# TaceoLabs/co-snarks

Hardware: NVIDIA H100
Metric: co-Groth16 proofs/sec (BN254, 2^20 constraints); MSM Mscalar/s (higher is better)
Workload: dtype u32x8 (256-bit Montgomery, integer)

## Files before the change

### co_snarks_b200/csrc/cs_groth16.cu

```cuda
#include <functional>
#include "cs_lib.cuh"
#include "cs_net.h"

using namespace cs;

struct cs_groth16_pk {
  int curve = 0;
  size_t nc = 0, ni = 0, nw = 0, n = 0;
  unsigned log_n = 0;
  DevBuf a_rowptr, a_col, a_coeff, b_rowptr, b_col, b_coeff;
  cs_bases *a_query = nullptr, *b_g1 = nullptr, *b_g2 = nullptr, *l_query = nullptr, *h_query = nullptr;
  std::vector<uint64_t> alpha_g1, beta_g1, beta_g2, delta_g1, delta_g2;
  std::vector<uint64_t> a_head, b1_head, b2_head;
  cs_domain* dom = nullptr;
  DevBuf coset_tab;
  DevBuf d_pub, d_wit, d_a, d_b, d_c, d_m1, d_m2;
  DevBuf c_rowptr, c_col, c_coeff;
  bool have_c = false;
  int wit_src[4] = {0, 1, 2, 3};
  cs_domain* dom_ark = nullptr;
  DevBuf coset_tab_ark, ginv_pows, vinv_over_n;
  DevBuf d_pt;
};

// ... 755 lines not shown

extern "C" {

int cs_groth16_rep3_prove(cs_ctx* ctx, cs_groth16_pk* pk, cs_net* net0, cs_net* net1, cs_rep3_state* state,
                          const uint64_t* h_pub, const uint64_t* h_wit, const uint64_t* d_wit, uint64_t* out_a,
                          uint64_t* out_b, uint64_t* out_c, uint64_t* out_rs) {
  return rep3_prove_dispatch(ctx, pk, net0, net1, nullptr, 0, state ? state->id : 0, state, h_pub, h_wit, d_wit, out_a, out_b,
                             out_c, out_rs);
}

int cs_groth16_rep3_prove_main(cs_ctx* ctx, cs_groth16_pk* pk, cs_net* net0, cs_net* net1, cs_net* pair,
                               cs_rep3_state* state, const uint64_t* h_pub, const uint64_t* h_wit, const uint64_t* d_wit,
                               uint64_t* out_a, uint64_t* out_b, uint64_t* out_c, uint64_t* out_rs) {
  return rep3_prove_dispatch(ctx, pk, net0, net1, pair, 1, state ? state->id : 0, state, h_pub, h_wit, d_wit, out_a, out_b,
                             out_c, out_rs);
}

int cs_groth16_rep3_prove_helper(cs_ctx* ctx, cs_groth16_pk* pk, int party, cs_net* pair, cs_rep3_state* state,
                                 const uint64_t* h_pub, const uint64_t* h_wit, const uint64_t* d_wit) {
  if (state && state->id != party) return fail(CS_ERR_ARG, "cs_groth16_rep3_prove_helper: state belongs to party %d", state->id);
  return rep3_prove_dispatch(ctx, pk, nullptr, nullptr, pair, 2, party, state, h_pub, h_wit, d_wit, nullptr, nullptr, nullptr,
                             nullptr);
}

int cs_groth16_pk_create(cs_ctx* ctx, const cs_groth16_key_desc* d, cs_groth16_pk** out) {
  return cs::groth16_pk_create(ctx, d, 0, out);
}

}

int cs::groth16_pk_create(cs_ctx* ctx, const cs_groth16_key_desc* d, unsigned k, cs_groth16_pk** out) {
  if (!ctx || !d || !out) return fail(CS_ERR_ARG, "cs_groth16_pk_create: NULL argument");
  if (d->curve != CS_BN254
#if defined(CS_ENABLE_BLS12_381)
      && d->curve != CS_BLS12_381
#endif
  )
    return fail(CS_ERR_ARG, "cs_groth16_pk_create: unsupported curve %d", (int)d->curve);
  const size_t nc = d->num_constraints, ni = d->num_instance_variables, nw = d->num_witness_variables;
  if (ni == 0) return fail(CS_ERR_ARG, "cs_groth16_pk_create: num_instance_variables must be >= 1");
  if (d->a_query_len != ni + nw || d->b_g1_query_len != ni + nw || d->b_g2_query_len != ni + nw)
    return fail(CS_ERR_ARG, "cs_groth16_pk_create: a/b query length must be %zu", ni + nw);
  if (d->l_query_len != nw) return fail(CS_ERR_ARG, "cs_groth16_pk_create: l_query length must be %zu", nw);
  if (d->window_bits && (d->window_bits < 2 || d->window_bits > (int)MSM_MAX_WINDOW))
    return fail(CS_ERR_ARG, "cs_bases_upload: window_bits %d out of range [2,%u] (0 = automatic)", d->window_bits, MSM_MAX_WINDOW);
  CS_CUDA(cudaSetDevice(ctx->device));
  std::unique_ptr<cs_groth16_pk, void (*)(cs_groth16_pk*)> pk(new cs_groth16_pk(), cs_groth16_pk_free);
  pk->curve = d->curve;
  pk->nc = nc; pk->ni = ni; pk->nw = nw;
  size_t n = 1;
  unsigned lg = 0;
  while (n < nc + ni) { n <<= 1; lg++; }
  pk->n = n;
  pk->log_n = lg;
  if (d->h_query_len < n) return fail(CS_ERR_ARG, "cs_groth16_pk_create: h_query has %zu points, domain needs %zu", d->h_query_len, n);
  const unsigned max_adicity = d->curve == CS_BN254 ? 28 : 32;
  if (lg > max_adicity) return fail(CS_ERR_ARG, "Polynomial Degree too large");
  const size_t fq = fq_limbs64(d->curve), g1b = 2 * fq * 8, g2b = 4 * fq * 8;
  CS_TRY(upload(ctx, pk->a_rowptr, d->a_row_ptr, (nc + 1) * 4));
  CS_TRY(upload(ctx, pk->a_col, d->a_col, d->a_nnz * 4));
  CS_TRY(upload(ctx, pk->a_coeff, d->a_coeff, d->a_nnz * 32));
  CS_TRY(upload(ctx, pk->b_rowptr, d->b_row_ptr, (nc + 1) * 4));
  CS_TRY(upload(ctx, pk->b_col, d->b_col, d->b_nnz * 4));
  CS_TRY(upload(ctx, pk->b_coeff, d->b_coeff, d->b_nnz * 32));
  if (d->c_row_ptr) {
    CS_TRY(upload(ctx, pk->c_rowptr, d->c_row_ptr, (nc + 1) * 4));
    CS_TRY(upload(ctx, pk->c_col, d->c_col, d->c_nnz * 4));
    CS_TRY(upload(ctx, pk->c_coeff, d->c_coeff, d->c_nnz * 32));
    pk->have_c = true;
  }
  CS_CUDA(cudaStreamSynchronize(ctx->stream));
  pk->alpha_g1.assign(d->alpha_g1, d->alpha_g1 + 2 * fq);
  pk->beta_g1.assign(d->beta_g1, d->beta_g1 + 2 * fq);
  pk->beta_g2.assign(d->beta_g2, d->beta_g2 + 4 * fq);
  pk->delta_g1.assign(d->delta_g1, d->delta_g1 + 2 * fq);
  pk->delta_g2.assign(d->delta_g2, d->delta_g2 + 4 * fq);
  pk->a_head.assign(d->a_query, d->a_query + ni * 2 * fq);
  pk->b1_head.assign(d->b_g1_query, d->b_g1_query + ni * 2 * fq);
  pk->b2_head.assign(d->b_g2_query, d->b_g2_query + ni * 4 * fq);
  (void)g1b; (void)g2b;
  const int wb = d->window_bits;
  int wwb = wb, hwb = wb;
  CS_DISPATCH_CURVE(d->curve, {
    if (!wwb) wwb = (int)msm_auto_window(nw, Cfg::FR_BITS);
    if (!hwb) hwb = (int)msm_auto_window(n, Cfg::FR_BITS);
    const unsigned cmax = wwb > hwb ? wwb : hwb;
    const unsigned W = msm_shape(Cfg::FR_BITS, wwb < hwb ? wwb : hwb).W;
    if (!k)
      CS_TRY(pick_table_rows(ctx, cmax, W, [&](unsigned kk) { return key_bytes<Cfg>(ni, nw, n, wwb, hwb, kk); },
                             "cs_groth16_pk_create", &k));
  });
  CS_TRY(bases_upload(ctx, d->curve, CS_G1, d->a_query, d->a_query_len, wwb, k, &pk->a_query));
  CS_TRY(bases_upload(ctx, d->curve, CS_G1, d->b_g1_query, d->b_g1_query_len, wwb, k, &pk->b_g1));
  CS_TRY(bases_upload(ctx, d->curve, CS_G2, d->b_g2_query, d->b_g2_query_len, wwb, k, &pk->b_g2));
  if (nw) CS_TRY(bases_upload(ctx, d->curve, CS_G1, d->l_query, d->l_query_len, wwb, k, &pk->l_query));
  CS_TRY(bases_upload(ctx, d->curve, CS_G1, d->h_query, n, hwb, k, &pk->h_query));
  CS_TRY(plan_witness_views(ctx, pk.get()));
  switch (d->curve) {
    case CS_BN254: CS_TRY(build_coset_table<Bn254Cfg>(ctx, pk.get())); break;
#if defined(CS_ENABLE_BLS12_381)
    case CS_BLS12_381: CS_TRY(build_coset_table<Bls381Cfg>(ctx, pk.get())); break;
#endif
    default: break;
  }
  *out = pk.release();
  return 0;
}

extern "C" {

void cs_groth16_pk_free(cs_groth16_pk* pk) {
  if (!pk) return;
  DevBuf* bufs[] = {&pk->a_rowptr, &pk->a_col, &pk->a_coeff, &pk->b_rowptr, &pk->b_col, &pk->b_coeff, &pk->coset_tab,
                    &pk->d_pub, &pk->d_wit, &pk->d_a, &pk->d_b, &pk->d_c, &pk->d_m1, &pk->d_m2,
                    &pk->c_rowptr, &pk->c_col, &pk->c_coeff, &pk->coset_tab_ark, &pk->ginv_pows, &pk->vinv_over_n,
                    &pk->d_pt};
  for (DevBuf* b : bufs) b->release();
  cs_bases_free(pk->a_query);
  cs_bases_free(pk->b_g1);
  cs_bases_free(pk->b_g2);
  cs_bases_free(pk->l_query);
  cs_bases_free(pk->h_query);
  cs_domain_free(pk->dom);
  cs_domain_free(pk->dom_ark);
  delete pk;
}

size_t cs_groth16_domain_size(const cs_groth16_pk* pk) { return pk ? pk->n : 0; }

int cs_groth16_pk_table_info(const cs_groth16_pk* pk, unsigned* table_rows, size_t* table_bytes) {
  if (!pk) return fail(CS_ERR_ARG, "cs_groth16_pk_table_info: pk is NULL");
  const cs_bases* q[5] = {pk->a_query, pk->b_g1, pk->b_g2, pk->l_query, pk->h_query};
  size_t bytes = 0;
  for (const cs_bases* b : q)
    if (b) bytes += b->table.cap + b->infmask.cap;
  if (table_rows) *table_rows = pk->a_query->sh.T;
  if (table_bytes) *table_bytes = bytes;
  return 0;
}
int cs_groth16_pk_curve(const cs_groth16_pk* pk) { return pk ? pk->curve : CS_ERR_ARG; }

int cs_groth16_witness_map(cs_ctx* ctx, cs_groth16_pk* pk, cs_share_kind kind, int party, const uint64_t* h_pub,
                           const uint64_t* h_wit, const uint64_t* h_m1, const uint64_t* h_m2, uint64_t* h_out) {
  if (!ctx || !pk || !h_pub || (pk->nw && !h_wit)) return fail(CS_ERR_ARG, "cs_groth16_witness_map: NULL argument");
  if (kind != CS_PLAIN && kind != CS_REP3) return fail(CS_ERR_ARG, "cs_groth16_witness_map: bad share kind");
  if (kind == CS_REP3 && (party < 0 || party > 2)) return fail(CS_ERR_ARG, "cs_groth16_witness_map: party must be 0..2");
  CS_CUDA(cudaSetDevice(ctx->device));
  CS_TRY(upload_inputs(ctx, pk, kind, h_pub, h_wit, h_m1, h_m2));
  switch (pk->curve) {
    case CS_BN254:
      CS_TRY((witness_map_device<Bn254Cfg>(ctx, pk, kind, party, pk->d_wit.as<uint32_t>(), h_m1 != nullptr,
                                           h_m2 != nullptr, ctx->stream)));
      break;
#if defined(CS_ENABLE_BLS12_381)
    case CS_BLS12_381:
      CS_TRY((witness_map_device<Bls381Cfg>(ctx, pk, kind, party, pk->d_wit.as<uint32_t>(), h_m1 != nullptr,
                                            h_m2 != nullptr, ctx->stream)));
      break;
#endif
    default: return fail(CS_ERR_ARG, "unsupported curve");
  }
  if (h_out) CS_CUDA(cudaMemcpyAsync(h_out, pk->d_c.p, pk->n * 32, cudaMemcpyDeviceToHost, ctx->stream));
  CS_CUDA(cudaStreamSynchronize(ctx->stream));
  return 0;
}

int cs_groth16_witness_map_libsnark(cs_ctx* ctx, cs_groth16_pk* pk, cs_share_kind kind, int party, const uint64_t* h_pub,
                                    const uint64_t* h_wit, const uint64_t* h_mask, uint64_t* h_out) {
// ... 187 lines not shown
```

### co_snarks_b200/csrc/cs_msm.cuh

```cuda
#pragma once
#include <stdlib.h>
#include "cs_common.cuh"
#include "cs_curve.cuh"

namespace cs {

constexpr unsigned MSM_SLICE_MAX = 64;
constexpr unsigned MSM_ORDER_BLOCK = 256;
constexpr unsigned MSM_RED_SEG = 4;
constexpr unsigned MSM_SIGN = 0x80000000u;

template <class FrP, class Fn>
CS_D void msm_recode(const uint32_t* __restrict__ scalars, uint32_t sstride, uint32_t i, int mont, uint32_t c,
                     uint32_t W, uint32_t k, Fn&& f) {
  Fp<FrP> s;
  const uint4* src = reinterpret_cast<const uint4*>(scalars) + (size_t)i * sstride * (FrP::N / 4);
  CS_UNROLL
  for (int q = 0; q < FrP::N / 4; q++) {
    uint4 v = src[q];
    s.l[4 * q] = v.x; s.l[4 * q + 1] = v.y; s.l[4 * q + 2] = v.z; s.l[4 * q + 3] = v.w;
  }
  if (mont) s = s.from_mont();
  const uint32_t half = 1u << (c - 1);
  const uint32_t mask = (1u << c) - 1;
  uint32_t carry = 0, row = 0, gb = 0;
  for (uint32_t w = 0; w < W; w++) {
    uint32_t pos = w * c;
    uint32_t li = pos >> 5, sh = pos & 31;
    uint32_t lo = li < FrP::N ? s.l[li] : 0;
    uint32_t hi = li + 1 < FrP::N ? s.l[li + 1] : 0;
    uint32_t d = (__funnelshift_r(lo, hi, sh) & mask) + carry;
    uint32_t out;
    if (d > half) {
      out = ((1u << c) - d) | MSM_SIGN;
      carry = 1;
    } else {
      out = d;
      carry = 0;
    }
    f(row, out & ~MSM_SIGN ? out + gb : 0);
    gb += half;
    if (gb == k * half) {
      gb = 0;
      row++;
    }
  }
}

CS_D bool msm_base_inf(const uint32_t* __restrict__ infmask, uint32_t k) {
  return infmask && ((infmask[k >> 5] >> (k & 31)) & 1);
}

constexpr unsigned MSM_BIN_T = 1024;
constexpr unsigned MSM_BIN_TILE = 4096;
constexpr unsigned MSM_BIN_SPAN = 1u << 15;
constexpr unsigned MSM_SCATTER_SPAN = 1u << 13;

template <class FrP>
CS_GLOBAL void __launch_bounds__(MSM_BIN_T) k_msm_bin_count(const uint32_t* __restrict__ scalars, uint32_t sstride,
                                                            uint32_t n, int mont, uint32_t c, uint32_t W, uint32_t kw,
                                                            const uint32_t* __restrict__ infmask, uint32_t offset,
                                                            uint32_t tile, uint32_t nblk_p, uint32_t pstride, uint32_t B,
                                                            uint32_t* __restrict__ tab) {
  CS_DYN_SMEM(uint32_t, h);
  const uint32_t bt = blockIdx.x % nblk_p;
  scalars += (size_t)(blockIdx.x / nblk_p) * pstride * FrP::N;
  const uint32_t lo = blockIdx.y * MSM_BIN_SPAN + 1;
  const uint32_t span = B + 1 - lo < MSM_BIN_SPAN ? B + 1 - lo : MSM_BIN_SPAN;
  for (uint32_t k = threadIdx.x; k < span; k += blockDim.x) h[k] = 0;
  __syncthreads();
  const uint32_t i1 = (bt + 1) * tile < n ? (bt + 1) * tile : n;
  for (uint32_t i = bt * tile + threadIdx.x; i < i1; i += blockDim.x) {
    if (msm_base_inf(infmask, offset + i)) continue;
    msm_recode<FrP>(scalars, sstride, i, mont, c, W, kw, [&](uint32_t, uint32_t d) {
      const uint32_t k = (d & ~MSM_SIGN) - lo;
      if (k < span) atomicAdd(&h[k], 1u);
    });
  }
  __syncthreads();
  uint32_t* row = tab + (size_t)blockIdx.x * B + (lo - 1);
  for (uint32_t k = threadIdx.x; k < span; k += blockDim.x) row[k] = h[k];
}

constexpr unsigned MSM_BIN_SCAN_U = 16;
static CS_GLOBAL void k_msm_bin_scan(uint32_t* __restrict__ tab, uint32_t nblk, uint32_t B, uint32_t NB,
                                     uint32_t* __restrict__ count) {
  const uint32_t b = blockIdx.x * blockDim.x + threadIdx.x;
  if (b == 0) count[0] = 0;
  if (b >= NB) return;
  uint32_t* col = tab + (size_t)(b / B) * nblk * B + b % B;
  uint32_t run = 0, r = 0;
  for (; r + MSM_BIN_SCAN_U <= nblk; r += MSM_BIN_SCAN_U) {
    uint32_t v[MSM_BIN_SCAN_U];
    CS_UNROLL
    for (uint32_t u = 0; u < MSM_BIN_SCAN_U; u++) v[u] = col[(size_t)(r + u) * B];
    CS_UNROLL
    for (uint32_t u = 0; u < MSM_BIN_SCAN_U; u++) {
      col[(size_t)(r + u) * B] = run;
      run += v[u];
    }
  }
  for (; r < nblk; r++) {
    const uint32_t v = col[(size_t)r * B];
    col[(size_t)r * B] = run;
    run += v;
  }
  count[b + 1] = run;
}

template <class FrP>
CS_GLOBAL void __launch_bounds__(MSM_BIN_T) k_msm_bin_scatter(const uint32_t* __restrict__ scalars, uint32_t sstride,
                                                              uint32_t n, int mont, uint32_t c, uint32_t W, uint32_t kw,
                                                              const uint32_t* __restrict__ infmask, uint32_t offset,
                                                              uint32_t tile, uint32_t nblk_p, uint32_t pstride,
                                                              uint32_t B, uint32_t nbases,
                                                              const uint32_t* __restrict__ tab,
                                                              const uint32_t* __restrict__ start,
                                                              uint32_t* __restrict__ sorted) {
  CS_DYN_SMEM(uint32_t, cur);
  const uint32_t p = blockIdx.x / nblk_p, bt = blockIdx.x % nblk_p;
  scalars += (size_t)p * pstride * FrP::N;
  const uint32_t lo = blockIdx.y * MSM_SCATTER_SPAN + 1;
  const uint32_t span = B + 1 - lo < MSM_SCATTER_SPAN ? B + 1 - lo : MSM_SCATTER_SPAN;
  const uint32_t* row = tab + (size_t)blockIdx.x * B + (lo - 1);
  for (uint32_t k = threadIdx.x; k < span; k += blockDim.x) cur[k] = start[p * B + lo + k] + row[k];
  __syncthreads();
  const uint32_t i1 = (bt + 1) * tile < n ? (bt + 1) * tile : n;
  for (uint32_t i = bt * tile + threadIdx.x; i < i1; i += blockDim.x) {
    if (msm_base_inf(infmask, offset + i)) continue;
    msm_recode<FrP>(scalars, sstride, i, mont, c, W, kw, [&](uint32_t row, uint32_t d) {
      const uint32_t k = (d & ~MSM_SIGN) - lo;
      if (k < span) sorted[atomicAdd(&cur[k], 1u)] = (row * nbases + offset + i) | (d & MSM_SIGN);
    });
  }
}

template <class F>
CS_GLOBAL void k_msm_infmask(const Affine<F>* __restrict__ table, uint32_t n, uint32_t* __restrict__ mask) {
  uint32_t wd = blockIdx.x * blockDim.x + threadIdx.x;
  if (wd * 32 >= n) return;
  uint32_t m = 0;
  for (uint32_t k = 0; k < 32 && wd * 32 + k < n; k++)
    if (table[wd * 32 + k].is_inf()) m |= 1u << k;
  mask[wd] = m;
}

constexpr unsigned MSM_SCAN_T = 1024;
constexpr unsigned MSM_SCAN_MAX_BLOCKS = 1024;
CS_D void msm_scan_terms(const uint32_t* __restrict__ count, uint32_t k, uint32_t nb1, uint32_t S, uint32_t* v) {
  uint32_t cnt = (k && k < nb1) ? count[k] : 0;
  uint32_t n0 = (cnt + S - 1) / S;
  uint32_t n1 = (n0 + S - 1) / S;
  v[0] = cnt; v[1] = n0; v[2] = n1; v[3] = (n1 + S - 1) / S;
}
static CS_GLOBAL void k_msm_scan1(const uint32_t* __restrict__ count, uint32_t nb1 , uint32_t S,
                                  uint32_t* __restrict__ start, uint32_t* __restrict__ sstart0,
                                  uint32_t* __restrict__ sstart1, uint32_t* __restrict__ sstart2, uint32_t* __restrict__ aux) {
  __shared__ uint32_t sm[4][32];
  const uint32_t t = threadIdx.x, lane = t & 31, wid = t >> 5, nwarp = blockDim.x >> 5;
  const uint32_t k = blockIdx.x * blockDim.x + t;
  uint32_t v[4], inc[4];
  msm_scan_terms(count, k, nb1, S, v);
  CS_UNROLL
  for (int q = 0; q < 4; q++) {
    uint32_t x = v[q];
    CS_UNROLL
    for (uint32_t d = 1; d < 32; d <<= 1) {
      uint32_t y = __shfl_up_sync(0xffffffffu, x, d);
      if (lane >= d) x += y;
    }
    inc[q] = x;
    if (lane == 31) sm[q][wid] = x;
  }
  __syncthreads();
  uint32_t w[4], x[4];
  CS_UNROLL
  for (int q = 0; q < 4; q++) {
    w[q] = (wid == 0 && lane < nwarp) ? sm[q][lane] : 0;
    x[q] = w[q];
    CS_UNROLL
    for (uint32_t d = 1; d < 32; d <<= 1) {
      uint32_t y = __shfl_up_sync(0xffffffffu, x[q], d);
      if (lane >= d) x[q] += y;
    }
  }
  __syncthreads();
  if (wid == 0 && lane < nwarp) {
    CS_UNROLL
    for (int q = 0; q < 4; q++) sm[q][lane] = x[q] - w[q];
    if (lane == nwarp - 1) {
      CS_UNROLL
      for (int q = 0; q < 4; q++) aux[blockIdx.x * 4 + q] = x[q];
    }
  }
  __syncthreads();
  if (k < nb1) {
    start[k] = sm[0][wid] + inc[0] - v[0];
    sstart0[k] = sm[1][wid] + inc[1] - v[1];
    sstart1[k] = sm[2][wid] + inc[2] - v[2];
    sstart2[k] = sm[3][wid] + inc[3] - v[3];
  }
}
static CS_GLOBAL void k_msm_scan2(const uint32_t* __restrict__ count, uint32_t nb1, uint32_t S,
                                  uint32_t* __restrict__ start, uint32_t* __restrict__ sstart0,
                                  uint32_t* __restrict__ sstart1, uint32_t* __restrict__ sstart2,
                                  const uint32_t* __restrict__ aux) {
  const uint32_t k = blockIdx.x * blockDim.x + threadIdx.x;
  if (k >= nb1) return;
  uint32_t off[4] = {0, 0, 0, 0};
  for (uint32_t b = 0; b < blockIdx.x; b++) {
    CS_UNROLL
    for (int q = 0; q < 4; q++) off[q] += aux[b * 4 + q];
  }
  uint32_t a = start[k] + off[0], b0 = sstart0[k] + off[1], b1 = sstart1[k] + off[2], b2 = sstart2[k] + off[3];
  start[k] = a; sstart0[k] = b0; sstart1[k] = b1; sstart2[k] = b2;
  if (k == nb1 - 1) {
    uint32_t v[4];
    msm_scan_terms(count, k, nb1, S, v);
    start[nb1] = a + v[0]; sstart0[nb1] = b0 + v[1]; sstart1[nb1] = b1 + v[2]; sstart2[nb1] = b2 + v[3];
  }
}

constexpr unsigned MSM_VIEW_T = 256;
constexpr unsigned MSM_VIEW_WORDS = MSM_VIEW_T / 32;

CS_D uint32_t popc32(uint32_t x) {
#if defined(CS_EMU)
  return (uint32_t)__builtin_popcount(x);
#else
  return __popc(x);
#endif
// ... 390 lines not shown

constexpr uint32_t POINT_INV_RUN = 32;

template <class F, class FrP>
CS_GLOBAL void __launch_bounds__(128) k_point_terms(const Affine<F>* __restrict__ base, const uint32_t* __restrict__ scalars,
                                                    uint32_t nterms, Xyzz<F>* __restrict__ prod) {
  const uint32_t t = blockIdx.x * blockDim.x + threadIdx.x;
  if (t >= nterms) return;
  Fp<FrP> s;
  CS_UNROLL
  for (int k = 0; k < FrP::N; k++) s.l[k] = scalars[(size_t)t * FrP::N + k];
  prod[t] = scalar_mul<F, FrP>(base[t], s.from_mont());
}

template <class F>
CS_GLOBAL void __launch_bounds__(128) k_point_sum(const Xyzz<F>* __restrict__ prod, uint32_t T, uint32_t nout,
                                                  const Xyzz<F>* __restrict__ add0, const Xyzz<F>* __restrict__ add1,
                                                  const Affine<F>* __restrict__ shared, Xyzz<F>* __restrict__ out) {
  const uint32_t o = blockIdx.x * blockDim.x + threadIdx.x;
  if (o >= nout) return;
  Xyzz<F> acc = shared ? Xyzz<F>::from_affine(*shared) : Xyzz<F>::inf();
  for (uint32_t j = 0; j < T + 2; j++) {
    const Xyzz<F>* q = j < T ? prod + (size_t)o * T + j : (j == T ? add0 : add1);
    if (q && j >= T) q += o;
    if (q) padd(acc, *q);
  }
  out[o] = acc;
}

template <class F>
CS_GLOBAL void __launch_bounds__(128) k_point_affine(const Xyzz<F>* __restrict__ in, uint32_t nout, uint32_t ostride,
                                                     Affine<F>* __restrict__ out) {
  const uint32_t lo = (blockIdx.x * blockDim.x + threadIdx.x) * POINT_INV_RUN;
  if (lo >= nout) return;
  const uint32_t hi = lo + POINT_INV_RUN < nout ? lo + POINT_INV_RUN : nout;
  F run = F::one();
  for (uint32_t o = lo; o < hi; o++) {
    if (!in[o].is_inf()) run = run * in[o].zzz;
    out[(size_t)o * ostride].x = run;
  }
  F inv = run.inverse();
  for (uint32_t o = hi; o-- > lo;) {
    Affine<F> a = Affine<F>::inf();
    if (!in[o].is_inf()) {
      const F zi = o > lo ? inv * out[(size_t)(o - 1) * ostride].x : inv;
      inv = inv * in[o].zzz;
      const F zzi = (zi * in[o].zz).sqr();
      a.x = in[o].x * zzi;
      a.y = in[o].y * zi;
    }
    out[(size_t)o * ostride] = a;
  }
}

struct MsmShape {
  uint32_t c, W, B;
  uint32_t k = 1, T = 0;
  uint32_t nb() const { return k * B; }
};

static inline MsmShape msm_shape(uint32_t scalar_bits, uint32_t c, uint32_t k = 1) {
  MsmShape s;
  s.c = c;
  s.W = (scalar_bits + 1 + c - 1) / c;
  s.B = 1u << (c - 1);
  s.k = k < s.W ? k : s.W;
  s.T = (s.W + s.k - 1) / s.k;
  return s;
}

static inline uint32_t msm_auto_window(size_t n, uint32_t scalar_bits) {
  int lg = 0;
  while ((1ull << (lg + 1)) <= n) lg++;
  int c = lg >= 15 ? 16 : lg - 4;
  if (c < 4) c = 4;
  while (c < 16) {
    const uint32_t W = (scalar_bits + 1 + c - 1) / c;
    const uint32_t top = scalar_bits + 1 - (W - 1) * c;
    if (2 * top >= (uint32_t)c) break;
    c++;
  }
  return (uint32_t)c;
}
static inline uint32_t msm_slice(const MsmShape& sh) {
  const char* e = getenv("CS_MSM_SLICE");
  if (e && atoi(e) == 64) return 64u;
  if (e && atoi(e) == 32) return 32u;
  return sh.c >= 18 ? 64u : 32u;
}

constexpr int MSM_NSTAGE = 5;
struct MsmWorkspace {
  DevBuf dig, sorted, meta, part0, part1, part2, bucket, red, scal, result, order;
  void* h_result = nullptr;
  size_t h_result_cap = 0;
  bool profile = false;
  cudaEvent_t ev[MSM_NSTAGE + 1] = {};
  cudaEvent_t sorted_ev = nullptr;
  bool sorted_ev_made = false, sorted_once = false;
  cudaEvent_t acc_in = nullptr, acc_out = nullptr;
  size_t bytes() const {
    return dig.cap + sorted.cap + meta.cap + part0.cap + part1.cap + part2.cap + bucket.cap + red.cap + scal.cap +
           result.cap + order.cap;
  }
  int mark(int i, cudaStream_t st) {
    if (!profile) return 0;
    if (!ev[i]) CS_CUDA(cudaEventCreateWithFlags(&ev[i], 0));
    CS_CUDA(cudaEventRecord(ev[i], st));
    return 0;
  }
  void release() {
    for (int i = 0; i <= MSM_NSTAGE; i++) {
      if (ev[i]) cudaEventDestroy(ev[i]);
      ev[i] = nullptr;
    }
    if (sorted_ev_made) cudaEventDestroy(sorted_ev);
    if (acc_in) cudaEventDestroy(acc_in);
    if (acc_out) cudaEventDestroy(acc_out);
    acc_in = acc_out = nullptr;
    sorted_ev = nullptr;
    sorted_ev_made = sorted_once = false;
    dig.release(); sorted.release(); meta.release(); part0.release(); part1.release(); part2.release();
    bucket.release(); red.release(); scal.release(); result.release(); order.release();
    if (h_result) cudaFreeHost(h_result);
    h_result = nullptr;
    h_result_cap = 0;
  }
};

template <class F>
int msm_accum0_f52(const Affine<F>* table, const uint32_t* sorted, const uint32_t* count, const uint32_t* start,
                   const uint32_t* sstart0, uint32_t nb1, uint32_t S, const uint32_t* order, const uint32_t* order_b,
                   Xyzz<F>* part0, uint32_t max_s0, cudaStream_t st);

struct MsmSizes {
  uint32_t nb1, S, ob, K;
  size_t nent, max_s0, max_s1, max_s2;
  MsmSizes(const MsmShape& sh, uint32_t n, uint32_t K_ = 1) {
    K = K_;
    nb1 = K * sh.nb() + 1;
    nent = (size_t)K * sh.W * n;
    S = msm_slice(sh);
    max_s0 = nent / S + nb1;
    max_s1 = max_s0 / S + nb1;
    max_s2 = max_s1 / S + nb1;
    ob = ceil_div(max_s0, MSM_ORDER_BLOCK);
  }
  size_t meta_words() const { return (size_t)nb1 + 4 * ((size_t)nb1 + 1) + 4 * MSM_SCAN_MAX_BLOCKS; }
  size_t order_words() const {
    return 4 * max_s0 + (size_t)ob * (MSM_SLICE_MAX + 1) + 2 * (MSM_SLICE_MAX + 1) + (size_t)(MSM_SLICE_MAX + 1) * MSM_OFF_CHUNKS;
  }
};
struct MsmSortBufs {
  uint32_t *count, *start, *sstart0, *sstart1, *sstart2, *aux;
  uint32_t *slice_len, *slice_bkt, *order, *order_b, *block_hist, *len_base, *chunk_sum;
  MsmSortBufs(const MsmWorkspace& w, const MsmSizes& z) {
    count = w.meta.as<uint32_t>();
    start = count + z.nb1;
    sstart0 = start + z.nb1 + 1;
    sstart1 = sstart0 + z.nb1 + 1;
    sstart2 = sstart1 + z.nb1 + 1;
    aux = sstart2 + z.nb1 + 1;
    slice_len = w.order.as<uint32_t>();
    slice_bkt = slice_len + z.max_s0;
    order = slice_bkt + z.max_s0;
    order_b = order + z.max_s0;
    block_hist = order_b + z.max_s0;
    len_base = block_hist + (size_t)z.ob * (MSM_SLICE_MAX + 1);
    chunk_sum = len_base + 2 * (MSM_SLICE_MAX + 1);
  }
};

static inline uint32_t msm_max_batch(const MsmShape& sh, uint32_t n) {
  size_t K = ((size_t)MSM_SCAN_MAX_BLOCKS * MSM_SCAN_T - 1) / sh.nb();
  if (n) K = K < ((1ull << 31) - 1) / ((size_t)sh.W * n) ? K : ((1ull << 31) - 1) / ((size_t)sh.W * n);
  K = K < 65535 / sh.k ? K : 65535 / sh.k;
  return (uint32_t)K;
}

static inline int msm_check_limits(const MsmShape& sh, uint32_t n, uint32_t nbases, uint32_t K = 1) {
  const size_t nent = (size_t)K * sh.W * n;
  if (nent >= (1ull << 31) || (size_t)sh.T * nbases >= (1ull << 31))
    return fail(-3, "msm: K*W*n = %zu entries or T*nbases = %zu table slots exceed 2^31", nent, (size_t)sh.T * nbases);
  if (K > 1 && K > msm_max_batch(sh, n))
    return fail(-3, "msm: a batch of %u MSMs exceeds the %u that one sort takes in this window shape (K*k*B + 1 <= 2^20 "
                    "buckets, K*k <= 65535 groups)", K, msm_max_batch(sh, n));
  return 0;
}

static inline int msm_scan(const MsmSortBufs& q, const MsmSizes& z, uint32_t NB, cudaStream_t st) {
  const uint32_t sb = ceil_div(z.nb1, MSM_SCAN_T);
  if (sb > MSM_SCAN_MAX_BLOCKS) return fail(-3, "msm: %u buckets exceed the scan's limit", NB);
  CS_LAUNCH_SYNC(k_msm_scan1, sb, MSM_SCAN_T, 0, st, q.count, z.nb1, z.S, q.start, q.sstart0, q.sstart1, q.sstart2, q.aux);
  CS_LAUNCH(k_msm_scan2, sb, MSM_SCAN_T, 0, st, q.count, z.nb1, z.S, q.start, q.sstart0, q.sstart1, q.sstart2, q.aux);
  return 0;
}

static inline int msm_slice_order(MsmWorkspace& ws, const MsmSortBufs& q, const MsmSizes& z, cudaStream_t st) {
  CS_LAUNCH_SYNC(k_msm_slice_hist, z.ob, MSM_ORDER_BLOCK, 0, st, q.count, q.sstart0, z.nb1, z.S, q.slice_len, q.slice_bkt,
                 q.block_hist);
  const uint32_t nt = (MSM_SLICE_MAX + 1) * MSM_OFF_CHUNKS;
  CS_LAUNCH(k_msm_slice_off1, ceil_div(nt, 128), 128, 0, st, q.block_hist, z.ob, q.chunk_sum);
  CS_LAUNCH(k_msm_slice_off2, 1, 128, 0, st, q.chunk_sum, q.len_base);
  CS_LAUNCH(k_msm_slice_off3, ceil_div(nt, 128), 128, 0, st, q.block_hist, z.ob, q.chunk_sum, q.len_base);
  CS_LAUNCH_SYNC(k_msm_slice_order, z.ob, MSM_ORDER_BLOCK, 0, st, q.slice_len, q.slice_bkt, (uint32_t)z.max_s0, q.sstart0,
                 z.nb1, q.block_hist, q.len_base, q.order, q.order_b);
  if (!ws.sorted_ev_made) {
    CS_CUDA(cudaEventCreateWithFlags(&ws.sorted_ev, cudaEventDisableTiming));
    ws.sorted_ev_made = true;
  }
  CS_CUDA(cudaEventRecord(ws.sorted_ev, st));
  ws.sorted_once = true;
  return 0;
}

template <class FrP>
int msm_smem_optin() {
#if !defined(CS_EMU)
  CS_CUDA(cudaFuncSetAttribute(k_msm_bin_count<FrP>, cudaFuncAttributeMaxDynamicSharedMemorySize, MSM_BIN_SPAN * 4));
  CS_CUDA(cudaFuncSetAttribute(k_msm_bin_scatter<FrP>, cudaFuncAttributeMaxDynamicSharedMemorySize, MSM_SCATTER_SPAN * 4));
#endif
  return 0;
}

static inline uint32_t msm_bin_tile(const MsmShape& sh, const MsmSizes& z, uint32_t n) {
  const size_t ent = z.nent / z.K;
  const size_t rows = ent / sh.nb() > 1 ? ent / sh.nb() : 1;
  const size_t nblk = ceil_div(n, MSM_BIN_TILE) < rows ? ceil_div(n, MSM_BIN_TILE) : rows;
  return n ? ceil_div(n, nblk) : 1;
}

static inline size_t msm_sort_dig_words(const MsmShape& sh, const MsmSizes& z, uint32_t n) {
  const size_t tab_words = (size_t)z.K * (n ? ceil_div(n, msm_bin_tile(sh, z, n)) : 0) * sh.nb();
  return tab_words > z.nent ? tab_words : z.nent;
}
static inline size_t msm_view_dig_words(const MsmSizes& z) {
  const size_t nblk = ceil_div(z.nent, MSM_VIEW_T);
  return nblk * MSM_VIEW_WORDS + 2 * nblk + 1;
}

template <class F>
struct MsmReduce {
  uint32_t L, nseg_g, nseg, ngroups, fs_threads, fs_blocks;
  size_t red_elems;
  explicit MsmReduce(const MsmShape& sh, uint32_t K = 1) {
    L = sh.B < MSM_RED_SEG ? sh.B : MSM_RED_SEG;
    nseg_g = sh.B / L;
    ngroups = K * sh.k;
    nseg = ngroups * nseg_g;
    fs_threads = sizeof(Xyzz<F>) > 128 ? 128 : 256;
    fs_blocks = nseg_g > 4 * fs_threads ? (nseg_g + fs_threads - 1) / fs_threads : 1;
    red_elems = (size_t)nseg + (size_t)ngroups * fs_blocks + (sh.k > 1 ? ngroups : 0);
  }
};

static inline size_t msm_sort_bytes(const MsmShape& sh, uint32_t n, uint32_t K = 1) {
  const MsmSizes z(sh, n, K);
  const size_t dig = msm_sort_dig_words(sh, z, n) > msm_view_dig_words(z) ? msm_sort_dig_words(sh, z, n) : msm_view_dig_words(z);
  return DevBuf::alloc_size(dig * 4) + DevBuf::alloc_size(z.nent * 4) + DevBuf::alloc_size(z.meta_words() * 4) +
         DevBuf::alloc_size(z.order_words() * 4);
}
template <class F>
size_t msm_accum_bytes(const MsmShape& sh, uint32_t n, uint32_t K = 1) {
  const MsmSizes z(sh, n, K);
  const size_t x = sizeof(Xyzz<F>);
  return DevBuf::alloc_size(z.max_s0 * x) + DevBuf::alloc_size(z.max_s1 * x) + DevBuf::alloc_size(z.max_s2 * x) +
         DevBuf::alloc_size((size_t)z.nb1 * x) + DevBuf::alloc_size(MsmReduce<F>(sh, K).red_elems * x) +
         DevBuf::alloc_size(K * x);
}

template <class FrP>
int msm_sort(MsmWorkspace& ws, const uint32_t* infmask, uint32_t nbases, MsmShape sh, uint32_t offset,
             const uint32_t* d_scalars, uint32_t sstride, uint32_t n, int mont, cudaStream_t st, uint32_t K = 1,
             uint32_t pstride = 0) {
  CS_TRY(msm_check_limits(sh, n, nbases, K));
  const MsmSizes z(sh, n, K);
  const uint32_t tile = msm_bin_tile(sh, z, n);
  const uint32_t nblk_p = n ? ceil_div(n, tile) : 0, nblk = K * nblk_p;
  const uint32_t NB = sh.nb();
  const dim3 grid(nblk, ceil_div(NB, MSM_BIN_SPAN)), grid_sc(nblk, ceil_div(NB, MSM_SCATTER_SPAN));
  const uint32_t smem = (NB < MSM_BIN_SPAN ? NB : MSM_BIN_SPAN) * 4;
  const uint32_t smem_sc = (NB < MSM_SCATTER_SPAN ? NB : MSM_SCATTER_SPAN) * 4;
  CS_TRY(ws.dig.reserve(msm_sort_dig_words(sh, z, n) * 4));
  CS_TRY(ws.sorted.reserve(z.nent * 4));
  CS_TRY(ws.meta.reserve(z.meta_words() * 4));
  CS_TRY(ws.order.reserve(z.order_words() * 4));
  const MsmSortBufs q(ws, z);
  uint32_t* tab = ws.dig.as<uint32_t>();
  CS_TRY(ws.mark(0, st));
  if (nblk)
    CS_LAUNCH_SYNC(k_msm_bin_count<FrP>, grid, MSM_BIN_T, smem, st, d_scalars, sstride, n, mont, sh.c, sh.W, sh.k,
                   infmask, offset, tile, nblk_p, pstride, NB, tab);
  CS_TRY(ws.mark(1, st));
  CS_LAUNCH(k_msm_bin_scan, ceil_div(K * NB, 256), 256, 0, st, tab, nblk_p, NB, K * NB, q.count);
  CS_TRY(msm_scan(q, z, K * NB, st));
  if (nblk)
    CS_LAUNCH_SYNC(k_msm_bin_scatter<FrP>, grid_sc, MSM_BIN_T, smem_sc, st, d_scalars, sstride, n, mont, sh.c, sh.W, sh.k,
                   infmask, offset, tile, nblk_p, pstride, NB, nbases, tab, q.start, ws.sorted.as<uint32_t>());
  return msm_slice_order(ws, q, z, st);
}

static inline int msm_view(MsmWorkspace& ws, const MsmWorkspace& src, const uint32_t* infmask, uint32_t nbases,
                           MsmShape sh, uint32_t offset, uint32_t n, cudaStream_t st, uint32_t K = 1) {
  const MsmSizes z(sh, n, K);
  const uint32_t nblk = ceil_div(z.nent, MSM_VIEW_T);
  CS_TRY(ws.dig.reserve(msm_view_dig_words(z) * 4));
  CS_TRY(ws.sorted.reserve(z.nent * 4));
  CS_TRY(ws.meta.reserve(z.meta_words() * 4));
  CS_TRY(ws.order.reserve(z.order_words() * 4));
  const MsmSortBufs q(ws, z), s(src, z);
  uint32_t* keep = ws.dig.as<uint32_t>();
  uint32_t* blk_cnt = keep + (size_t)nblk * MSM_VIEW_WORDS;
  uint32_t* blk_off = blk_cnt + nblk;
  const uint32_t* src_sorted = src.sorted.as<uint32_t>();
  CS_LAUNCH_SYNC(k_msm_view_flags, nblk, MSM_VIEW_T, 0, st, src_sorted, s.start, z.nb1, n, infmask, offset, keep, blk_cnt);
  CS_LAUNCH_SYNC(k_msm_view_scan, 1, MSM_SCAN_T, 0, st, blk_cnt, nblk, blk_off);
  CS_LAUNCH(k_msm_view_counts, ceil_div(z.nb1, 256), 256, 0, st, s.start, z.nb1, keep, blk_off, q.count);
  CS_LAUNCH(k_msm_view_scatter, nblk, MSM_VIEW_T, 0, st, src_sorted, n, nbases, offset, keep, blk_off,
            ws.sorted.as<uint32_t>());
  CS_TRY(msm_scan(q, z, K * sh.nb(), st));
  return msm_slice_order(ws, q, z, st);
}

template <class F, class FrP>
int msm_enqueue(MsmWorkspace& ws, const Affine<F>* table, const uint32_t* infmask, uint32_t nbases, MsmShape sh,
                uint32_t offset,
                const uint32_t* d_scalars, uint32_t sstride, uint32_t n, int mont, cudaStream_t st,
                MsmWorkspace* sort_from = nullptr, bool view = false, bool table_m260 = false, cudaStream_t st_acc = nullptr,
                uint32_t K = 1, uint32_t pstride = 0) {
  CS_TRY(msm_check_limits(sh, n, nbases, K));
  const MsmSizes z(sh, n, K);
  const uint32_t nb1 = z.nb1, S = z.S;
  const size_t max_s0 = z.max_s0, max_s1 = z.max_s1, max_s2 = z.max_s2;
  CS_TRY(ws.part0.reserve(max_s0 * sizeof(Xyzz<F>)));
  CS_TRY(ws.part1.reserve(max_s1 * sizeof(Xyzz<F>)));
  CS_TRY(ws.part2.reserve(max_s2 * sizeof(Xyzz<F>)));
  CS_TRY(ws.bucket.reserve((size_t)nb1 * sizeof(Xyzz<F>)));
  const MsmReduce<F> rd(sh, K);
  const uint32_t L = rd.L, nseg = rd.nseg, fs_threads = rd.fs_threads, fs_blocks = rd.fs_blocks, G = rd.ngroups;
  CS_TRY(ws.red.reserve(rd.red_elems * sizeof(Xyzz<F>)));
  CS_TRY(ws.result.reserve(K * sizeof(Xyzz<F>)));
  if (ws.h_result_cap < K * sizeof(Xyzz<F>)) {
    if (ws.h_result) cudaFreeHost(ws.h_result);
    ws.h_result = nullptr;
    ws.h_result_cap = 0;
    CS_CUDA(cudaMallocHost(&ws.h_result, K * sizeof(Xyzz<F>)));
    ws.h_result_cap = K * sizeof(Xyzz<F>);
  }
  if (sort_from) {
    if (!sort_from->sorted_once) return fail(-1, "msm: the workspace to share a sort with has not been enqueued");
    CS_TRY(ws.mark(0, st));
    CS_CUDA(cudaStreamWaitEvent(st, sort_from->sorted_ev, 0));
    CS_TRY(ws.mark(1, st));
    if (view) CS_TRY(msm_view(ws, *sort_from, infmask, nbases, sh, offset, n, st, K));
  } else {
    CS_TRY(msm_sort<FrP>(ws, infmask, nbases, sh, offset, d_scalars, sstride, n, mont, st, K, pstride));
  }
  MsmWorkspace& so = sort_from && !view ? *sort_from : ws;
  const MsmSortBufs q(so, z);
  const uint32_t *count = q.count, *start = q.start, *sstart0 = q.sstart0, *sstart1 = q.sstart1, *sstart2 = q.sstart2;
  const uint32_t *order = q.order, *order_b = q.order_b;
  CS_TRY(ws.mark(2, st));
  cudaStream_t st_main = st;
  if (st_acc) {
    if (!ws.acc_in) {
      CS_CUDA(cudaEventCreateWithFlags(&ws.acc_in, cudaEventDisableTiming));
      CS_CUDA(cudaEventCreateWithFlags(&ws.acc_out, cudaEventDisableTiming));
    }
    CS_CUDA(cudaEventRecord(ws.acc_in, st));
    CS_CUDA(cudaStreamWaitEvent(st_acc, ws.acc_in, 0));
    st = st_acc;
  }
  {
    static int minb_env = -1;
    if (minb_env < 0) { const char* e = getenv("CS_ACCUM0_MINB"); minb_env = e ? atoi(e) : 0; }
    const int minb = minb_env ? minb_env : (sizeof(Affine<F>) > 64 ? 2 : 4);
    if (table_m260) {
      CS_TRY((msm_accum0_f52<F>(table, so.sorted.as<uint32_t>(), count, start, sstart0, nb1, S, order, order_b,
                                ws.part0.as<Xyzz<F>>(), (uint32_t)max_s0, st)));
    } else {
#define CS_ACC0(M)                                                                                              \
// ... 47 lines not shown
```

Measured before the change: 51.66.

## Use 17-bit MSM windows for large keys with 16-bit packed bin counters

For key MSMs of at least 2^18 points where auto-selection picks c=16, the window becomes 17 bits when that reduces the window count. For BN254 this means 15 windows instead of 16. To fit the doubled bucket range in shared memory, the bin count kernel packs two 16-bit counters per word, with the tile capped so counts cannot overflow. The scatter span, scan block limit and reduction segment length are also widened to handle more buckets. The trade is fewer windows and bucket passes against larger bucket reductions, bigger precomputed tables and more shared-memory atomics contention.

```diff
diff --git a/co_snarks_b200/csrc/cs_groth16.cu b/co_snarks_b200/csrc/cs_groth16.cu
--- a/co_snarks_b200/csrc/cs_groth16.cu
+++ b/co_snarks_b200/csrc/cs_groth16.cu
@@ -861,8 +861,8 @@
   const int wb = d->window_bits;
   int wwb = wb, hwb = wb;
   CS_DISPATCH_CURVE(d->curve, {
-    if (!wwb) wwb = (int)msm_auto_window(nw, Cfg::FR_BITS);
-    if (!hwb) hwb = (int)msm_auto_window(n, Cfg::FR_BITS);
+    if (!wwb) wwb = (int)msm_key_window(nw, Cfg::FR_BITS);
+    if (!hwb) hwb = (int)msm_key_window(n, Cfg::FR_BITS);
     const unsigned cmax = wwb > hwb ? wwb : hwb;
     const unsigned W = msm_shape(Cfg::FR_BITS, wwb < hwb ? wwb : hwb).W;
     if (!k)
diff --git a/co_snarks_b200/csrc/cs_msm.cuh b/co_snarks_b200/csrc/cs_msm.cuh
--- a/co_snarks_b200/csrc/cs_msm.cuh
+++ b/co_snarks_b200/csrc/cs_msm.cuh
@@ -8,6 +8,7 @@
 constexpr unsigned MSM_SLICE_MAX = 64;
 constexpr unsigned MSM_ORDER_BLOCK = 256;
 constexpr unsigned MSM_RED_SEG = 4;
+constexpr unsigned MSM_RED_MAX_SEG = 1u << 13;
 constexpr unsigned MSM_SIGN = 0x80000000u;
 
 template <class FrP, class Fn>
@@ -54,32 +55,40 @@
 constexpr unsigned MSM_BIN_T = 1024;
 constexpr unsigned MSM_BIN_TILE = 4096;
 constexpr unsigned MSM_BIN_SPAN = 1u << 15;
+constexpr unsigned MSM_BIN_SPAN16 = 1u << 16;
 constexpr unsigned MSM_SCATTER_SPAN = 1u << 13;
+constexpr unsigned MSM_SCATTER_SPAN_MAX = 1u << 14;
+
+static inline uint32_t msm_scatter_span(uint32_t NB) { return NB > MSM_BIN_SPAN ? MSM_SCATTER_SPAN_MAX : MSM_SCATTER_SPAN; }
 
 template <class FrP>
 CS_GLOBAL void __launch_bounds__(MSM_BIN_T) k_msm_bin_count(const uint32_t* __restrict__ scalars, uint32_t sstride,
                                                             uint32_t n, int mont, uint32_t c, uint32_t W, uint32_t kw,
                                                             const uint32_t* __restrict__ infmask, uint32_t offset,
                                                             uint32_t tile, uint32_t nblk_p, uint32_t pstride, uint32_t B,
-                                                            uint32_t* __restrict__ tab) {
+                                                            uint32_t h16, uint32_t* __restrict__ tab) {
   CS_DYN_SMEM(uint32_t, h);
   const uint32_t bt = blockIdx.x % nblk_p;
   scalars += (size_t)(blockIdx.x / nblk_p) * pstride * FrP::N;
-  const uint32_t lo = blockIdx.y * MSM_BIN_SPAN + 1;
-  const uint32_t span = B + 1 - lo < MSM_BIN_SPAN ? B + 1 - lo : MSM_BIN_SPAN;
-  for (uint32_t k = threadIdx.x; k < span; k += blockDim.x) h[k] = 0;
+  const uint32_t hspan = h16 ? MSM_BIN_SPAN16 : MSM_BIN_SPAN;
+  const uint32_t lo = blockIdx.y * hspan + 1;
+  const uint32_t span = B + 1 - lo < hspan ? B + 1 - lo : hspan;
+  for (uint32_t k = threadIdx.x; k < (h16 ? (span + 1) >> 1 : span); k += blockDim.x) h[k] = 0;
   __syncthreads();
   const uint32_t i1 = (bt + 1) * tile < n ? (bt + 1) * tile : n;
   for (uint32_t i = bt * tile + threadIdx.x; i < i1; i += blockDim.x) {
     if (msm_base_inf(infmask, offset + i)) continue;
     msm_recode<FrP>(scalars, sstride, i, mont, c, W, kw, [&](uint32_t, uint32_t d) {
       const uint32_t k = (d & ~MSM_SIGN) - lo;
-      if (k < span) atomicAdd(&h[k], 1u);
+      if (k < span) {
+        if (h16) atomicAdd(&h[k >> 1], 1u << ((k & 1) << 4));
+        else atomicAdd(&h[k], 1u);
+      }
     });
   }
   __syncthreads();
   uint32_t* row = tab + (size_t)blockIdx.x * B + (lo - 1);
-  for (uint32_t k = threadIdx.x; k < span; k += blockDim.x) row[k] = h[k];
+  for (uint32_t k = threadIdx.x; k < span; k += blockDim.x) row[k] = h16 ? (h[k >> 1] >> ((k & 1) << 4)) & 0xffffu : h[k];
 }
 
 constexpr unsigned MSM_BIN_SCAN_U = 16;
@@ -113,15 +122,15 @@
                                                               uint32_t n, int mont, uint32_t c, uint32_t W, uint32_t kw,
                                                               const uint32_t* __restrict__ infmask, uint32_t offset,
                                                               uint32_t tile, uint32_t nblk_p, uint32_t pstride,
-                                                              uint32_t B, uint32_t nbases,
+                                                              uint32_t B, uint32_t nbases, uint32_t sspan,
                                                               const uint32_t* __restrict__ tab,
                                                               const uint32_t* __restrict__ start,
                                                               uint32_t* __restrict__ sorted) {
   CS_DYN_SMEM(uint32_t, cur);
   const uint32_t p = blockIdx.x / nblk_p, bt = blockIdx.x % nblk_p;
   scalars += (size_t)p * pstride * FrP::N;
-  const uint32_t lo = blockIdx.y * MSM_SCATTER_SPAN + 1;
-  const uint32_t span = B + 1 - lo < MSM_SCATTER_SPAN ? B + 1 - lo : MSM_SCATTER_SPAN;
+  const uint32_t lo = blockIdx.y * sspan + 1;
+  const uint32_t span = B + 1 - lo < sspan ? B + 1 - lo : sspan;
   const uint32_t* row = tab + (size_t)blockIdx.x * B + (lo - 1);
   for (uint32_t k = threadIdx.x; k < span; k += blockDim.x) cur[k] = start[p * B + lo + k] + row[k];
   __syncthreads();
@@ -146,7 +155,7 @@
 }
 
 constexpr unsigned MSM_SCAN_T = 1024;
-constexpr unsigned MSM_SCAN_MAX_BLOCKS = 1024;
+constexpr unsigned MSM_SCAN_MAX_BLOCKS = 2048;
 CS_D void msm_scan_terms(const uint32_t* __restrict__ count, uint32_t k, uint32_t nb1, uint32_t S, uint32_t* v) {
   uint32_t cnt = (k && k < nb1) ? count[k] : 0;
   uint32_t n0 = (cnt + S - 1) / S;
@@ -703,6 +712,12 @@
   }
   return (uint32_t)c;
 }
+
+static inline uint32_t msm_key_window(size_t n, uint32_t scalar_bits) {
+  const uint32_t c = msm_auto_window(n, scalar_bits);
+  if (n < (1u << 18) || c != 16) return c;
+  return (scalar_bits + 1 + 16) / 17 < (scalar_bits + 1 + 15) / 16 ? 17u : 16u;
+}
 static inline uint32_t msm_slice(const MsmShape& sh) {
   const char* e = getenv("CS_MSM_SLICE");
   if (e && atoi(e) == 64) return 64u;
@@ -804,7 +819,7 @@
   if (nent >= (1ull << 31) || (size_t)sh.T * nbases >= (1ull << 31))
     return fail(-3, "msm: K*W*n = %zu entries or T*nbases = %zu table slots exceed 2^31", nent, (size_t)sh.T * nbases);
   if (K > 1 && K > msm_max_batch(sh, n))
-    return fail(-3, "msm: a batch of %u MSMs exceeds the %u that one sort takes in this window shape (K*k*B + 1 <= 2^20 "
+    return fail(-3, "msm: a batch of %u MSMs exceeds the %u that one sort takes in this window shape (K*k*B + 1 <= 2^21 "
                     "buckets, K*k <= 65535 groups)", K, msm_max_batch(sh, n));
   return 0;
 }
@@ -839,16 +854,19 @@
 int msm_smem_optin() {
 #if !defined(CS_EMU)
   CS_CUDA(cudaFuncSetAttribute(k_msm_bin_count<FrP>, cudaFuncAttributeMaxDynamicSharedMemorySize, MSM_BIN_SPAN * 4));
-  CS_CUDA(cudaFuncSetAttribute(k_msm_bin_scatter<FrP>, cudaFuncAttributeMaxDynamicSharedMemorySize, MSM_SCATTER_SPAN * 4));
+  CS_CUDA(cudaFuncSetAttribute(k_msm_bin_scatter<FrP>, cudaFuncAttributeMaxDynamicSharedMemorySize, MSM_SCATTER_SPAN_MAX * 4));
 #endif
   return 0;
 }
+
+static inline bool msm_count16(const MsmShape& sh) { return sh.nb() > MSM_BIN_SPAN && sh.nb() <= MSM_BIN_SPAN16; }
 
 static inline uint32_t msm_bin_tile(const MsmShape& sh, const MsmSizes& z, uint32_t n) {
   const size_t ent = z.nent / z.K;
   const size_t rows = ent / sh.nb() > 1 ? ent / sh.nb() : 1;
   const size_t nblk = ceil_div(n, MSM_BIN_TILE) < rows ? ceil_div(n, MSM_BIN_TILE) : rows;
-  return n ? ceil_div(n, nblk) : 1;
+  const uint32_t tile = n ? ceil_div(n, nblk) : 1;
+  return msm_count16(sh) && tile > 65535 / sh.T ? 65535 / sh.T : tile;
 }
 
 static inline size_t msm_sort_dig_words(const MsmShape& sh, const MsmSizes& z, uint32_t n) {
@@ -865,7 +883,7 @@
   uint32_t L, nseg_g, nseg, ngroups, fs_threads, fs_blocks;
   size_t red_elems;
   explicit MsmReduce(const MsmShape& sh, uint32_t K = 1) {
-    L = sh.B < MSM_RED_SEG ? sh.B : MSM_RED_SEG;
+    L = sh.B < MSM_RED_SEG ? sh.B : sh.B / MSM_RED_SEG > MSM_RED_MAX_SEG ? sh.B / MSM_RED_MAX_SEG : MSM_RED_SEG;
     nseg_g = sh.B / L;
     ngroups = K * sh.k;
     nseg = ngroups * nseg_g;
@@ -899,9 +917,11 @@
   const uint32_t tile = msm_bin_tile(sh, z, n);
   const uint32_t nblk_p = n ? ceil_div(n, tile) : 0, nblk = K * nblk_p;
   const uint32_t NB = sh.nb();
-  const dim3 grid(nblk, ceil_div(NB, MSM_BIN_SPAN)), grid_sc(nblk, ceil_div(NB, MSM_SCATTER_SPAN));
-  const uint32_t smem = (NB < MSM_BIN_SPAN ? NB : MSM_BIN_SPAN) * 4;
-  const uint32_t smem_sc = (NB < MSM_SCATTER_SPAN ? NB : MSM_SCATTER_SPAN) * 4;
+  const bool h16 = msm_count16(sh);
+  const uint32_t hspan = h16 ? MSM_BIN_SPAN16 : MSM_BIN_SPAN, sspan = msm_scatter_span(NB);
+  const dim3 grid(nblk, ceil_div(NB, hspan)), grid_sc(nblk, ceil_div(NB, sspan));
+  const uint32_t smem = (h16 ? ceil_div(NB < hspan ? NB : hspan, 2) : (NB < hspan ? NB : hspan)) * 4;
+  const uint32_t smem_sc = (NB < sspan ? NB : sspan) * 4;
   CS_TRY(ws.dig.reserve(msm_sort_dig_words(sh, z, n) * 4));
   CS_TRY(ws.sorted.reserve(z.nent * 4));
   CS_TRY(ws.meta.reserve(z.meta_words() * 4));
@@ -911,13 +931,13 @@
   CS_TRY(ws.mark(0, st));
   if (nblk)
     CS_LAUNCH_SYNC(k_msm_bin_count<FrP>, grid, MSM_BIN_T, smem, st, d_scalars, sstride, n, mont, sh.c, sh.W, sh.k,
-                   infmask, offset, tile, nblk_p, pstride, NB, tab);
+                   infmask, offset, tile, nblk_p, pstride, NB, (uint32_t)h16, tab);
   CS_TRY(ws.mark(1, st));
   CS_LAUNCH(k_msm_bin_scan, ceil_div(K * NB, 256), 256, 0, st, tab, nblk_p, NB, K * NB, q.count);
   CS_TRY(msm_scan(q, z, K * NB, st));
   if (nblk)
     CS_LAUNCH_SYNC(k_msm_bin_scatter<FrP>, grid_sc, MSM_BIN_T, smem_sc, st, d_scalars, sstride, n, mont, sh.c, sh.W, sh.k,
-                   infmask, offset, tile, nblk_p, pstride, NB, nbases, tab, q.start, ws.sorted.as<uint32_t>());
+                   infmask, offset, tile, nblk_p, pstride, NB, nbases, sspan, tab, q.start, ws.sorted.as<uint32_t>());
   return msm_slice_order(ws, q, z, st);
 }
 
```

Result: faster. 53.00 (median of 6 runs) (+2.6%).
